# brucechin/OctopusZK

Measured on AMD Instinct MI355X. Metric: BN254 G1 VariableBaseMSM Mscalar-mul/s at 2^20, higher is better.
Workload: dtype u32; 1 GPU; VariableBaseMSM BN254 G1 2^20 random scalars/bases per GPU, bit-exact vs the serial CPU path (BASELINE.json configs[1]); n_per_gpu=1048576, window_bits=16, windows=8, glv=True, prepared_bases=False, msms_in_flight=3, schedule=pipeline3, parallelism=index-range shard x1, RCCL all-gather of 192-B partials + HIP point sum

## Files before the change

### octopuszk_amd/csrc/msm_var.cuh

```cuda
#pragma once
#include "curve.cuh"
#include "glv.cuh"

namespace ozk {

constexpr u32 BID_NONE = 0xffffffffu;

struct MsmPlan {
  int n_in;
  int glv;
  int n;
  int sd;
  int c;
  int cb;
  int W;
  int L1;
  int LK;
  int S;
};

OZK_HD u32 scalar_digit(const u32 (&s)[8], int w, int c) {
  const int bit = w * c;
  const int wi = bit >> 5, sh = bit & 31;
  u32 v = s[wi] >> sh;
// ... 693 lines not shown
    return IO::load_aff(w);
  }
  __device__ __forceinline__ void start_signed(const Aff<EA>& q, bool negate) {
    Aff<EA> qs = q;
    qs.y = select_el(negate, EA(reduce_to<17>(neg(q.y))), q.y);
    a = xyzz_from_affine<CV>(qs);
  }
  __device__ __forceinline__ void accumulate_signed(const Aff<EA>& q, bool negate) { a = xyzz_madd_lazy(a, q, negate); }
  __device__ __forceinline__ void store(u32* dst) const { IO::store_rec_xyzz(a, dst); }
  __device__ __forceinline__ void negate() { a.Y = typename CV::XY(reduce_to<32>(neg(reduce_to<32>(a.Y)))); }
  __device__ __forceinline__ void store_infinity(u32* dst) const {
    Xyzz<CV> z = a;
    z.ZZ = typename CV::XZZ(el_zero(z.ZZ));
    z.ZZZ = typename CV::XZZZ(el_zero(z.ZZ));
    IO::store_rec_xyzz(z, dst);
  }
};

template <class CV>
struct RunAccLds {
  using IO = CurveIO<CV>;
  using EA = typename CV::EA;
  static constexpr int RW = IO::RW;
  static constexpr int LDS_WORDS = 4 * RW;
  u32* col;
  template <class E>
  __device__ __forceinline__ E ld(int c) const {
    u32 w[RW];
#pragma unroll
    for (int k = 0; k < RW; k++) w[k] = col[(size_t)(c * RW + k) * 256];
    return ElemTraits<E>::load_raw(w);
  }
  template <class E>
  __device__ __forceinline__ void st(int c, const E& e) const {
    u32 w[RW];
    ElemTraits<E>::store_raw(e, w);
#pragma unroll
    for (int k = 0; k < RW; k++) col[(size_t)(c * RW + k) * 256] = w[k];
  }
  __device__ __forceinline__ void init(u32* lds) { col = lds + threadIdx.x; }
  __device__ __forceinline__ void put(const Xyzz<CV>& a) const {
    st(0, a.X);
    st(1, a.Y);
    st(2, a.ZZ);
    st(3, a.ZZZ);
  }
  static __device__ __forceinline__ Aff<EA> load_signed(const u32* pts, const u32* idx, long long p) {
    return RunAcc<CV, true>::load_signed(pts, idx, p);
  }
  using Raw = typename RunAcc<CV, true>::Raw;
  static __device__ __forceinline__ Raw load_raw(const u32* pts, u32 v) { return RunAcc<CV, true>::load_raw(pts, v); }
  static __device__ __forceinline__ __amdgpu_buffer_rsrc_t table_rsrc(const u32* pts) { return RunAcc<CV, true>::table_rsrc(pts); }
  static __device__ __forceinline__ Raw load_raw_buf(__amdgpu_buffer_rsrc_t rs, u32 v) { return RunAcc<CV, true>::load_raw_buf(rs, v); }
  static __device__ __forceinline__ Aff<EA> decode(const Raw& r, u32 v) { return RunAcc<CV, true>::decode(r, v); }
  __device__ __forceinline__ void start(const u32* pts, const u32* idx, long long p) {
    start_q(load_signed(pts, idx, p));
  }
  __device__ __forceinline__ void accumulate(const u32* pts, const u32* idx, long long p) {
    accumulate_q(load_signed(pts, idx, p));
  }
  __device__ __forceinline__ void start_q(const Aff<EA>& q) { put(xyzz_from_affine<CV>(q)); }
  __device__ __forceinline__ void accumulate_q(const Aff<EA>& q) {
    if (is_inf(q)) return;
    const auto ZZ = ld<typename CV::XZZ>(2);
    if (is_zero(ZZ)) {
      put(xyzz_from_affine<CV>(q));
      return;
    }
    if constexpr (CV::LAZY_FQ2) {
      const auto U2 = mul_lz(q.x, ZZ);
      const auto P = sub(U2, ld<typename CV::XX>(0));
      const auto ZZZ = ld<typename CV::XZZZ>(3);
      const auto R = sub(mul_lz(q.y, ZZZ), ld<typename CV::XY>(1));
      if (is_zero(P)) {
        if (is_zero(R)) {
          put(xyzz_dbl_affine<CV>(q));
        } else {
          st(2, typename CV::XZZ(el_zero(q.x)));
          st(3, typename CV::XZZZ(el_zero(q.x)));
        }
        return;
      }
      const auto Pr = reduce_to<32>(P);
      const auto PP = sqr_lz(Pr);
      const auto PPP = mul_lz(Pr, PP);
      st(2, typename CV::XZZ(mul_lz(ZZ, PP)));
      st(3, typename CV::XZZZ(mul_lz(ZZZ, PPP)));
      asm volatile("" ::: "memory");
      const auto Q = mul_lz(reduce_to<32>(ld<typename CV::XX>(0)), PP);
      const auto X3 = sub_sub2(sqr_lz(reduce_to<32>(R)), PPP, Q);
      st(0, typename CV::XX(X3));
      asm volatile("" ::: "memory");
      const auto Y3 = mulsub_lz(reduce_to<32>(R), reduce_to<32>(sub(Q, X3)), ld<typename CV::XY>(1), PPP);
      st(1, typename CV::XY(Y3));
      return;
    }
    const auto U2 = mul(q.x, ZZ);
    const auto P = sub(U2, ld<typename CV::XX>(0));
    const auto ZZZ = ld<typename CV::XZZZ>(3);
    const auto R = sub(mul(q.y, ZZZ), ld<typename CV::XY>(1));
    if (is_zero(P)) {
      if (is_zero(R)) {
        put(xyzz_dbl_affine<CV>(q));
      } else {
        st(2, typename CV::XZZ(el_zero(q.x)));
        st(3, typename CV::XZZZ(el_zero(q.x)));
      }
      return;
    }
    const auto PP = sqr(P);
    const auto PPP = mul(P, PP);
    st(2, typename CV::XZZ(mul(ZZ, PP)));
    st(3, typename CV::XZZZ(mul(ZZZ, PPP)));
    asm volatile("" ::: "memory");
    const auto Q = mul(ld<typename CV::XX>(0), PP);
    const auto X3 = sub(sqr(R), add(PPP, dbl(Q)));
    st(0, typename CV::XX(X3));
    asm volatile("" ::: "memory");
    const auto Y3 = mulsub(R, sub(Q, X3), ld<typename CV::XY>(1), PPP);
    st(1, typename CV::XY(Y3));
  }
  __device__ __forceinline__ Xyzz<CV> get() const {
    Xyzz<CV> a;
    a.X = ld<typename CV::XX>(0);
    a.Y = ld<typename CV::XY>(1);
    a.ZZ = ld<typename CV::XZZ>(2);
    a.ZZZ = ld<typename CV::XZZZ>(3);
    return a;
  }
  __device__ __forceinline__ void store(u32* dst) const { IO::store_rec_xyzz(get(), dst); }
  __device__ __forceinline__ void negate() const {
    st(1, typename CV::XY(reduce_to<32>(neg(reduce_to<32>(ld<typename CV::XY>(1))))));
  }
  __device__ __forceinline__ void store_infinity(u32* dst) const {
    Xyzz<CV> z = get();
    z.ZZ = typename CV::XZZ(el_zero(z.ZZ));
    z.ZZZ = typename CV::XZZZ(el_zero(z.ZZ));
    IO::store_rec_xyzz(z, dst);
  }
};
template <class CV>
struct RunAcc<CV, false> {
  using IO = CurveIO<CV>;
  Jac<CV> a;
  __device__ __forceinline__ void start(const u32* pts, const u32*, long long p) {
    a = IO::load_rec(pts + (size_t)p * IO::REC_WORDS);
  }
  __device__ __forceinline__ void accumulate(const u32* pts, const u32*, long long p) {
    a = jac_add(a, IO::load_rec(pts + (size_t)p * IO::REC_WORDS));
  }
  __device__ __forceinline__ void store(u32* dst) const { IO::store_rec_jac(a, dst); }
};

template <class CV, bool FIRST, bool LAZY = false>
__device__ __forceinline__ void
segreduce_lane(const int t, const u32* __restrict__ bid_in, const u32* __restrict__ idx_in,
               const u32* __restrict__ pts_in,
               const u32* __restrict__ d_count, int n_in_static, int L,
               u32* __restrict__ buckets, u32* __restrict__ bid_out, u32* __restrict__ pts_out) {
  using IO = CurveIO<CV>;
  if (!FIRST && *d_count == 0) return;
  const long long n_in = FIRST ? (long long)(*d_count) : (long long)n_in_static;
  const uint2* ent = reinterpret_cast<const uint2*>(idx_in);
  auto bid_at = [&](long long p) -> u32 {
    if constexpr (FIRST) return ent[p].y;
    else return bid_in[p];
  };
  const long long s = (long long)t * L;
  u32 head_bid = BID_NONE, tail_bid = BID_NONE;
  bool live = s < n_in;
  if (!FIRST && live) {
    const long long e0 = (s + L < n_in) ? (s + L) : n_in;
    bool any = false;
    for (long long p = s; p < e0; p++) any = any || (bid_in[p] != BID_NONE);
    live = any;
  }
  if (live) {
    const long long e = (s + L < n_in) ? (s + L) : n_in;
    const u32 first_bid = bid_at(s);
    const bool cb = (s > 0) && (bid_at(s - 1) == first_bid) && (first_bid != BID_NONE);
    const u32 last_bid = bid_at(e - 1);
    const bool cf = (e < n_in) && (bid_at(e) == last_bid) && (last_bid != BID_NONE);
    u32 cur = BID_NONE;
    bool cur_cb = false;
    using Acc = std::conditional_t<(FIRST && CV::LDS_ACC), RunAccLds<CV>, RunAcc<CV, FIRST>>;
    Acc acc;
    if constexpr (FIRST && CV::LDS_ACC) {
      extern __shared__ u32 ozk_acc_lds[];
      acc.init(ozk_acc_lds);
    }
    if constexpr (FIRST) {
      const u32 n_e = (u32)(e - s);
      const uint2* ent_c = ent + s;
      const uint2 e_first = ent_c[0];
      uint2 e_next = ent_c[n_e > 1 ? 1 : 0];
      u32 v_cur = e_first.x;
      const __amdgpu_buffer_rsrc_t table = Acc::table_rsrc(pts_in);
      typename Acc::Raw r = Acc::load_raw_buf(table, v_cur);
      u32 b_cur = first_bid;
      for (u32 k = 0; k < n_e; k++) {
        const u32 b = b_cur;
        const bool negate = (v_cur & SIDX_NEG) != 0;
        const auto q = [&] {
          if constexpr (LAZY) return Acc::decode_unsigned(r);
          else return Acc::decode(r, v_cur);
        }();
        const u32 k2 = (k + 2 < n_e) ? k + 2 : n_e - 1;
        const uint2 en = e_next;
        r = Acc::load_raw_buf(table, en.x);
        b_cur = en.y;
        v_cur = en.x;
        e_next = ent_c[k2];
        if (b != cur) {
          if (cur != BID_NONE) {
            if (cur_cb) {
              head_bid = cur;
              acc.store(pts_out + (size_t)(2 * (size_t)t) * IO::REC_WORDS);
            } else {
              acc.store(buckets + (size_t)cur * IO::REC_WORDS);
            }
          }
          cur = b;
          cur_cb = (k == 0) && cb;
          if constexpr (LAZY) acc.start_signed(q, negate);
          else acc.start_q(q);
        } else {
          if constexpr (LAZY) acc.accumulate_signed(q, negate);
          else acc.accumulate_q(q);
        }
      }
    } else {
    for (long long p = s; p < e; p++) {
      const u32 b = bid_in[p];
      if (b != cur) {
        if (cur != BID_NONE) {
          if (cur_cb) {
            head_bid = cur;
            acc.store(pts_out + (size_t)(2 * (size_t)t) * IO::REC_WORDS);
          } else {
            acc.store(buckets + (size_t)cur * IO::REC_WORDS);
          }
        }
        cur = b;
        cur_cb = (p == s) && cb;
        if (b != BID_NONE) acc.start(pts_in, idx_in, p);
      } else if (b != BID_NONE) {
        acc.accumulate(pts_in, idx_in, p);
      }
    }
    }
    if (cur != BID_NONE) {
      if (cur_cb) {
        head_bid = cur;
        acc.store(pts_out + (size_t)(2 * (size_t)t) * IO::REC_WORDS);
        if (cf) {
          tail_bid = cur;
          if constexpr (FIRST) {
            acc.store_infinity(pts_out + (size_t)(2 * (size_t)t + 1) * IO::REC_WORDS);
          } else {
            IO::store_rec_jac(jac_infinity<CV>(), pts_out + (size_t)(2 * (size_t)t + 1) * IO::REC_WORDS);
          }
        }
      } else if (cf) {
        tail_bid = cur;
        acc.store(pts_out + (size_t)(2 * (size_t)t + 1) * IO::REC_WORDS);
      } else {
        acc.store(buckets + (size_t)cur * IO::REC_WORDS);
      }
    }
  }
  bid_out[2 * (size_t)t] = head_bid;
  bid_out[2 * (size_t)t + 1] = tail_bid;
}

template <class CV, bool FIRST, bool LAZY = false>
__global__ void __launch_bounds__(256, (FIRST && CV::LDS_ACC) ? 2 : 1)
k_segreduce(const u32* __restrict__ bid_in, const u32* __restrict__ idx_in, const u32* __restrict__ pts_in,
            const u32* __restrict__ d_count, int n_in_static, int L,
            u32* __restrict__ buckets, u32* __restrict__ bid_out, u32* __restrict__ pts_out,
            int n_lanes, unsigned long long* __restrict__ clk) {
  const int t = blockIdx.x * blockDim.x + threadIdx.x;
  unsigned long long w0 = 0, c0 = 0;
  if constexpr (FIRST) {
    if (clk != nullptr && threadIdx.x == 0) {
      w0 = (unsigned long long)wall_clock64();
      c0 = (unsigned long long)clock64();
      atomicMax(&clk[0], ~w0);
    }
  }
  if (t < n_lanes)
    segreduce_lane<CV, FIRST, LAZY>(t, bid_in, idx_in, pts_in, d_count, n_in_static, L, buckets, bid_out, pts_out);
  if constexpr (FIRST) {
    if (clk != nullptr && (threadIdx.x & 63) == 0) {
      const unsigned long long w1 = (unsigned long long)wall_clock64();
      atomicMax(&clk[1], w1);
      if (threadIdx.x == 0) {
        atomicAdd(&clk[2], (unsigned long long)clock64() - c0);
        atomicAdd(&clk[3], w1 - w0);
      }
    }
  }
}

static __global__ void k_read_clock(unsigned long long* out) { out[0] = (unsigned long long)wall_clock64(); }

template <class CV>
__global__ void __launch_bounds__(256)
k_segreduce_small(const u32* __restrict__ d_count, int n_in, int L, u32* __restrict__ buckets,
                  u32* __restrict__ bid_a, u32* __restrict__ pts_a, u32* __restrict__ bid_b, u32* __restrict__ pts_b) {
  if (*d_count == 0) return;
  u32 *bi = bid_a, *pi = pts_a, *bo = bid_b, *po = pts_b;
  while (true) {
    const int lanes = (n_in + L - 1) / L;
    for (int t = threadIdx.x; t < lanes; t += blockDim.x)
      segreduce_lane<CV, false>(t, bi, nullptr, pi, d_count, n_in, L, buckets, bo, po);
    if (lanes == 1) break;
    block_sync();
    n_in = 2 * lanes;
    u32* tb = bi; bi = bo; bo = tb;
    u32* tp = pi; pi = po; po = tp;
  }
}

constexpr int RUN_MAX = 16;
template <class CV>
__global__ void __launch_bounds__(256)
k_runmerge(const u32* __restrict__ bid_in, const u32* __restrict__ pts, int n_slots,
           u32* __restrict__ buckets, u32* __restrict__ bid_out, u32* __restrict__ remaining) {
  using IO = CurveIO<CV>;
  const int t = blockIdx.x * blockDim.x + threadIdx.x;
  u32 alive = 0;
#pragma unroll 1
  for (int k = 0; k < 2; k++) {
    const int x = 2 * t + 1 + k;
    if (x >= n_slots) break;
    const u32 bx = bid_in[x];
    u32 out = BID_NONE;
    if (bx != BID_NONE) {
      int s = x, e = x;
      while (s > 0 && x - s < RUN_MAX && bid_in[s - 1] == bx) s--;
      while (e + 1 < n_slots && e - x < RUN_MAX && bid_in[e + 1] == bx) e++;
      const bool is_short = (x - s < RUN_MAX) && (e - x < RUN_MAX) && (e - s + 1 <= RUN_MAX);
      if (!is_short) {
        out = bx;
      } else if (s == x) {
        Xyzz<CV> acc = IO::load_xyzz(pts + (size_t)s * IO::REC_WORDS);
        for (int q = s + 1; q <= e; q += 2) acc = xyzz_add(acc, IO::load_xyzz(pts + (size_t)q * IO::REC_WORDS));
        IO::store_rec_xyzz(acc, buckets + (size_t)bx * IO::REC_WORDS);
      }
    }
    bid_out[x] = out;
    alive += (out != BID_NONE);
  }
  if (t == 0 && n_slots > 0) {
    bid_out[0] = bid_in[0];
    alive += (bid_in[0] != BID_NONE);
  }
  for (int o = 32; o > 0; o >>= 1) alive += __shfl_xor(alive, o);
  if ((threadIdx.x & 63) == 0 && alive) atomicAdd(remaining, alive);
}

template <class CV, bool FIRSTLEVEL>
__global__ void __launch_bounds__(256)
k_wsum(const u32* __restrict__ A_in, const u32* __restrict__ R_in, const u32* __restrict__ hist,
       int m_in, int S, int g, u32* __restrict__ A_out, u32* __restrict__ R_out, int m_out, int W, int prio) {
  using IO = CurveIO<CV>;
  if (prio) __builtin_amdgcn_s_setprio(3);
  const int t = blockIdx.x * blockDim.x + threadIdx.x;
  if (t >= m_out * W) return;
  const int w = t / m_out, j = t - w * m_out;
  const size_t base = (size_t)w * m_in;
  const int lo = j * S;
  int hi = lo + S;
  if (hi > m_in) hi = m_in;
  Jac<CV> run = jac_infinity<CV>(), ws = jac_infinity<CV>(), asum = jac_infinity<CV>();
  for (int e = hi - 1; e >= lo; e--) {
    if constexpr (FIRSTLEVEL) {
      if (hist[base + e] != 0) run = jac_add(run, IO::load_rec(R_in + (base + e) * IO::REC_WORDS));
    } else {
      run = jac_add(run, IO::load_jac(R_in + (base + e) * IO::JAC_WORDS));
    }
    if (e > lo) ws = jac_add(ws, run);
    if constexpr (!FIRSTLEVEL) asum = jac_add(asum, IO::load_jac(A_in + (base + e) * IO::JAC_WORDS));
  }
  for (int k = 0; k < g; k++) ws = jac_dbl(ws);
  if constexpr (!FIRSTLEVEL) ws = jac_add(ws, asum);
  IO::store_jac(ws, A_out + ((size_t)w * m_out + j) * IO::JAC_WORDS);
  IO::store_jac(run, R_out + ((size_t)w * m_out + j) * IO::JAC_WORDS);
}

template <class CV>
__device__ __forceinline__ Jac<CV> shfl_down_jac(const Jac<CV>& p, int o) {
  Jac<CV> r;
  r.X = shfl_down_el(p.X, o);
  r.Y = shfl_down_el(p.Y, o);
  r.Z = shfl_down_el(p.Z, o);
  return r;
}

template <class CV>
__device__ __forceinline__ void wave_combine(Jac<CV>& A, Jac<CV>& T, int l, int valid, int g) {
  for (int o = 1; o < valid; o <<= 1) {
    const Jac<CV> t = shfl_down_jac(T, o);
    const Jac<CV> s = jac_add(T, t);
    if (l + o < 64) T = s;
  }
  Jac<CV> U = T;
  for (int k = 0; k < g; k++) U = jac_dbl(U);
  const Jac<CV> AV = jac_add(A, U);
  Jac<CV> V = (l >= 1) ? AV : A;
  int top = 1;
  while (top < valid) top <<= 1;
  for (int o = top >> 1; o > 0; o >>= 1) {
    const Jac<CV> v = shfl_down_jac(V, o);
    const Jac<CV> s = jac_add(V, v);
    if (l < o) V = s;
  }
  A = V;
}

template <class CV>
__global__ void __launch_bounds__(64)
k_wsum_wave(const u32* __restrict__ A_in, const u32* __restrict__ R_in, int m_in, int g,
            u32* __restrict__ A_out, u32* __restrict__ R_out, int m_out, int W) {
  using IO = CurveIO<CV>;
  __builtin_amdgcn_s_setprio(3);
  const int wave = blockIdx.x;
  if (wave >= m_out * W) return;
  const int w = wave / m_out, j = wave - w * m_out;
  const int l = threadIdx.x & 63;
  const int e = j * 64 + l;
  int valid = m_in - j * 64;
  if (valid > 64) valid = 64;
  Jac<CV> A = jac_infinity<CV>(), T = jac_infinity<CV>();
  if (e < m_in) {
    A = IO::load_jac(A_in + ((size_t)w * m_in + e) * IO::JAC_WORDS);
    T = IO::load_jac(R_in + ((size_t)w * m_in + e) * IO::JAC_WORDS);
  }
  wave_combine<CV>(A, T, l, valid, g);
  if (l == 0) {
    IO::store_jac(A, A_out + ((size_t)w * m_out + j) * IO::JAC_WORDS);
    IO::store_jac(T, R_out + ((size_t)w * m_out + j) * IO::JAC_WORDS);
  }
}

template <class CV>
__global__ void __launch_bounds__(64)
k_wsum_fused(const u32* __restrict__ buckets, const u32* __restrict__ hist, int m_in, int S, int sg,
             u32* __restrict__ A_out, u32* __restrict__ R_out, int m_out, int W, int prio) {
  using IO = CurveIO<CV>;
  if (prio) __builtin_amdgcn_s_setprio(3);
  const int wave = blockIdx.x;
// ... 210 lines not shown
```

### octopuszk_amd/csrc/msm_var_driver.cuh

```cuda
#pragma once
#include <hip/hip_ext.h>
#include <pthread.h>
#include <stdlib.h>

#include <atomic>
#include <vector>

#ifndef OZK_WITH_G2
#define OZK_WITH_G2 1
#endif
#include "msm_var.cuh"
#include "host_ctx.h"
#include "fq2.cuh"

namespace ozk {

enum { PROF_OFF = 0, PROF_EVENTS = 1, PROF_CLOCK = 2 };
struct ProfState {
  pthread_mutex_t mu = PTHREAD_MUTEX_INITIALIZER;
  std::atomic<int> mode{PROF_OFF};
  int src = PROF_EVENTS;
  int every = 1, seen = 0;
  int count = 0;
  std::vector<hipEvent_t> e0, e1;
// ... 206 lines not shown
    rb->sorted = (a.off + 255) & ~(size_t)255;
    rb->sort_ws = (b.off + 255) & ~(size_t)255;
    rb->accum_ws = (c.off + 255) & ~(size_t)255;
  }
  L.bytes = a.off + b.off + c.off;
  return L;
}
template <class CV>
RegionBytes region_bytes(int n) {
  RegionBytes rb;
  make_layout3<CV>(plan_for<CV>(n), nullptr, nullptr, nullptr, &rb);
  return rb;
}

template <class CV>
size_t tail_layout(const MsmPlan& p, MsmLayout& L, void* tail, size_t tail_bytes) {
  using IO = CurveIO<CV>;
  Bump b(tail, tail_bytes);
  L.NB = (size_t)p.W << p.cb;
  L.m1 = (((size_t)1 << p.cb) + p.S - 1) / p.S;
  L.buckets = b.take<u32>(L.NB * IO::REC_WORDS);
  L.hist_t = b.take<u32>(L.NB);
  for (int k = 0; k < 2; k++) {
    L.wA[k] = b.take<u32>((size_t)p.W * L.m1 * IO::JAC_WORDS);
    L.wR[k] = b.take<u32>((size_t)p.W * L.m1 * IO::JAC_WORDS);
  }
  b.take<u32>(64);
  return b.off;
}

enum { TAIL_LATENCY = 0, TAIL_THROUGHPUT = 1 };
struct TailShape {
  bool fused;
  int serial_above;
};
static TailShape tail_shape(int mode) {
  const int forced = env_int("OZK_MSM_TAIL_MODE", -1);
  if (forced == 0 || forced == 1) mode = forced;
  TailShape t;
  t.fused = env_int("OZK_MSM_WSUM_FUSED", mode == TAIL_THROUGHPUT ? 0 : 1) != 0;
  t.serial_above = env_int("OZK_MSM_TAIL_SERIAL_ABOVE", mode == TAIL_THROUGHPUT ? 64 : (1 << 30));
  return t;
}
static void first_level_shape(const MsmPlan& p, bool fused, int* m_out, int* g_out) {
  const int m_in = 1 << p.cb;
  const int nseg = (m_in + p.S - 1) / p.S;
  const int sg = ilog2((uint32_t)p.S);
  if (fused) {
    *m_out = (nseg + 63) / 64;
    *g_out = sg + 6;
  } else {
    *m_out = nseg;
    *g_out = sg;
  }
}
template <class CV>
void launch_wsum0(const MsmPlan& p, const MsmLayout& L, hipStream_t st, int prio, bool fused) {
  const int TB = 256;
  const int m_in = 1 << p.cb;
  int m_out, g;
  first_level_shape(p, fused, &m_out, &g);
  const int tot = m_out * p.W;
  if (fused)
    hipLaunchKernelGGL((k_wsum_fused<CV>), dim3(tot), dim3(64), 0, st, L.buckets, L.hist_t, m_in, p.S,
                       ilog2((uint32_t)p.S), L.wA[0], L.wR[0], m_out, p.W, prio);
  else
    hipLaunchKernelGGL((k_wsum<CV, true>), dim3((tot + TB - 1) / TB), dim3(TB), 0, st, (const u32*)nullptr,
                       L.buckets, L.hist_t, m_in, p.S, 0, L.wA[0], L.wR[0], m_out, p.W, prio);
}

template <class CV>
int var_msm_sort(const void* d_bases, const void* d_scalars, int n, void* sorted, size_t sorted_bytes,
                        void* sort_ws, size_t sort_ws_bytes, hipStream_t st, hipEvent_t order_ev = nullptr,
                        const void* prepared = nullptr) {
  hip_clear_stale();
  const MsmPlan p = plan_for<CV>(n);
  if (prepared && p.glv && !p.sd) return fail(OZK_E_INVALID, "prepared bases need the signed-digit plan");
  RegionBytes rb;
  const MsmLayout L = make_layout3<CV>(p, sorted, sort_ws, nullptr, &rb, prepared);
  if (rb.sorted > sorted_bytes || rb.sort_ws > sort_ws_bytes)
    return fail(OZK_E_INVALID, "sort buffers too small: need %zu + %zu bytes, got %zu + %zu", rb.sorted, rb.sort_ws,
                sorted_bytes, sort_ws_bytes);
  const int TB = 256;
  const u32* bases = (const u32*)d_bases;
  const u32* scalars = (const u32*)d_scalars;
  const int n_in = p.n_in;
  n = p.n;
  OZK_HIP(hipMemsetAsync(L.total, 0, 4 * sizeof(u32), st));
  if (p.glv) {
    hipLaunchKernelGGL(k_digits_glv, dim3((n_in + TB - 1) / TB), dim3(TB), 0, st, scalars, n_in, p.c, p.W, p.sd,
                       L.digits, L.neg_flags);
    if (!prepared)
      hipLaunchKernelGGL((k_convert_bases<CV>), dim3((n_in + TB - 1) / TB), dim3(TB), 0, st, bases, L.aff, n_in, 1,
                         p.sd ? (const uint8_t*)nullptr : (const uint8_t*)L.neg_flags);
  } else {
    if (!prepared)
      hipLaunchKernelGGL((k_convert_bases<CV>), dim3((n_in + TB - 1) / TB), dim3(TB), 0, st, bases, L.aff, n_in, 0,
                         (const uint8_t*)nullptr);
    hipLaunchKernelGGL(k_digits, dim3((n_in + TB - 1) / TB), dim3(TB), 0, st, scalars, n_in, p.c, p.W, L.digits);
  }
  if (n <= SORTS_MAX_N && p.cb <= SORTS_MAX_CB && env_int("OZK_MSM_SMALL_SORT", 1)) {
    hipLaunchKernelGGL(k_sort_small, dim3(p.W), dim3(SORTS_BLOCK), 0, st, L.digits, n, p.cb, p.sd, L.total, L.hist, L.sent);
    if (order_ev && env_int("OZK_MSM_ORDER", 1)) OZK_HIP(hipStreamWaitEvent(st, order_ev, 0));
    OZK_HIP(hipGetLastError());
    return OZK_OK;
  }
  const size_t lds1 = (size_t)L.NH * sizeof(u32);
  hipLaunchKernelGGL(k_sort1_count, dim3(L.nblk, p.W), dim3(SORT_BLOCK), lds1, st, L.digits, n, L.lo_bits, p.sd,
                     L.NH, L.nblk, L.C1);
  const int items = SCAN_BLOCK * SCAN_ITEMS;
  const int nb = (int)((L.nC1 + items - 1) / items);
  hipLaunchKernelGGL(k_scan_blocksum, dim3(nb), dim3(SCAN_BLOCK), 0, st, L.C1, (int)L.nC1, L.blocksum);
  hipLaunchKernelGGL(k_scan_top, dim3(1), dim3(1024), 0, st, L.blocksum, nb, L.total);
  hipLaunchKernelGGL(k_scan_final, dim3(nb), dim3(SCAN_BLOCK), 0, st, L.C1, (int)L.nC1, L.blocksum, L.P1);
  const size_t lds_sc = ((size_t)2 * L.NH + 2 * SORT_CHUNK) * sizeof(u32);
  hipLaunchKernelGGL(k_sort1_scatter, dim3(L.nblk, p.W), dim3(SORT_BLOCK), lds_sc, st, L.digits, n, L.lo_bits,
                     p.sd, L.NH, L.nblk, L.P1, L.total, L.nC1, L.coarse);
  const int nbins = p.W * L.NH;
  const u32 sign_bit = p.sd ? 0x80u : 0u;
  const u32 big_thresh = (u32)(n / 64) > SORT_BIG ? (u32)(n / 64) : SORT_BIG;
  if (L.cap / ((size_t)big_thresh + 1) > (size_t)SORTBIG_MAXBINS)
    return fail(OZK_E_INVALID, "window plan c=%d (W=%d) at n=%d can produce more than %d oversized sort bins",
                p.c, p.W, p.n_in, SORTBIG_MAXBINS);
  hipLaunchKernelGGL(k_sort2, dim3(nbins), dim3(SORT2_BLOCK), 0, st, L.coarse, L.P1, L.total, p.cb, L.lo_bits, L.NH,
                     sign_bit, L.nblk, nbins, big_thresh, L.hist, L.sent);
  if (order_ev && env_int("OZK_MSM_ORDER", 1)) OZK_HIP(hipStreamWaitEvent(st, order_ev, 0));
  hipLaunchKernelGGL(k_sortbig_list, dim3(1), dim3(256), 0, st, L.P1, L.total, L.nblk, nbins, big_thresh, L.bigbins);
  hipLaunchKernelGGL(k_sortbig_count, dim3(1024), dim3(SORT_BLOCK), 0, st, L.coarse, L.bigbins,
                     (1u << L.lo_bits) - 1u, L.bigT);
  hipLaunchKernelGGL(k_sortbig_scan, dim3(SORTBIG_MAXBINS), dim3(256), 0, st, L.bigbins, L.bigT, p.cb, L.lo_bits, L.NH,
                     L.hist);
  hipLaunchKernelGGL(k_sortbig_scatter, dim3(1024), dim3(SORT_BLOCK), 0, st, L.coarse, L.bigbins, L.bigT, p.cb,
                     L.lo_bits, sign_bit, L.NH, L.sent);
  OZK_HIP(hipGetLastError());
  return OZK_OK;
}

enum { ACCUM_ALL = 0, ACCUM_LEVEL1 = 1, ACCUM_REST = 2 };
template <class CV>
int var_msm_accum(int n, void* sorted, size_t sorted_bytes, void* accum_ws, size_t accum_ws_bytes, void* tail,
                         size_t tail_bytes, hipStream_t st, const void* prepared = nullptr, int part = ACCUM_ALL) {
  hip_clear_stale();
  using CT = CV;
  const MsmPlan p = plan_for<CV>(n);
  RegionBytes rb;
  MsmLayout L = make_layout3<CV>(p, sorted, nullptr, accum_ws, &rb, prepared);
  if (rb.sorted > sorted_bytes || rb.accum_ws > accum_ws_bytes)
    return fail(OZK_E_INVALID, "accumulate buffers too small: need %zu + %zu bytes, got %zu + %zu", rb.sorted,
                rb.accum_ws, sorted_bytes, accum_ws_bytes);
  const size_t tneed = tail_layout<CV>(p, L, tail, tail_bytes);
  if (tneed > tail_bytes) return fail(OZK_E_INVALID, "tail buffer too small: need %zu bytes, got %zu", tneed, tail_bytes);
  const int TB = 256;
  size_t lanes = (L.cap + p.L1 - 1) / p.L1;
  if (part != ACCUM_REST) {
  hipEvent_t prof_e0 = nullptr, prof_e1 = nullptr;
  unsigned long long* clk = nullptr;
  g_prof.claim(&prof_e0, &prof_e1, &clk);
  const bool prof = prof_e0 != nullptr;
  size_t acc_lds = CV::LDS_ACC ? (size_t)RunAccLds<CV>::LDS_WORDS * TB * sizeof(u32) : 0;
  if (!CV::LDS_ACC) acc_lds = (size_t)env_int("OZK_L1_LDS", 41216);
  auto launch_l1 = [&](auto kern) {
    if (acc_lds > 65536)
      OZK_HIP(hipFuncSetAttribute((const void*)kern, hipFuncAttributeMaxDynamicSharedMemorySize, (int)acc_lds));
    hipExtLaunchKernelGGL(kern, dim3((unsigned)((lanes + TB - 1) / TB)), dim3(TB), (uint32_t)acc_lds, st,
                          prof ? prof_e0 : (hipEvent_t) nullptr, prof ? prof_e1 : (hipEvent_t) nullptr, 0u,
                          (const u32*)nullptr, (const u32*)L.sent, (const u32*)L.aff, (const u32*)L.total, 0, p.L1,
                          L.buckets, L.slot_bid[0], L.slot_pts[0], (int)lanes, clk);
    return OZK_OK;
  };
  int rc_l1;
  if constexpr (CV::LAZY_MADD) {
    if (env_int("OZK_L1_LAZY", 1)) rc_l1 = launch_l1(k_segreduce<CV, true, true>);
    else rc_l1 = launch_l1(k_segreduce<CV, true, false>);
  } else {
    rc_l1 = launch_l1(k_segreduce<CV, true, false>);
  }
  if (rc_l1) return rc_l1;
  }
  if (part == ACCUM_LEVEL1) {
    OZK_HIP(hipGetLastError());
    return OZK_OK;
  }
  size_t n_in = 2 * lanes;
  hipLaunchKernelGGL((k_runmerge<CT>), dim3((unsigned)((lanes + TB - 1) / TB)), dim3(TB), 0, st, L.slot_bid[0],
                     L.slot_pts[0], (int)n_in, L.buckets, L.slot_bid2, L.total + 1);
  int cur = 0;
  bool first_generic = true;
  const int small_lanes = env_int("OZK_MSM_SMALL_LEVEL_LANES", 1024);
  while (true) {
    lanes = (n_in + p.LK - 1) / p.LK;
    if (!first_generic && (int)lanes <= small_lanes) {
      hipLaunchKernelGGL((k_segreduce_small<CT>), dim3(1), dim3(TB), 0, st, L.total + 1, (int)n_in, p.LK, L.buckets,
                         L.slot_bid[cur], L.slot_pts[cur], L.slot_bid[cur ^ 1], L.slot_pts[cur ^ 1]);
      break;
    }
    hipLaunchKernelGGL((k_segreduce<CT, false>), dim3((unsigned)((lanes + TB - 1) / TB)), dim3(TB), 0, st,
                       first_generic ? L.slot_bid2 : L.slot_bid[cur], (const u32*)nullptr, L.slot_pts[cur],
                       L.total + 1, (int)n_in, p.LK, L.buckets, L.slot_bid[cur ^ 1], L.slot_pts[cur ^ 1], (int)lanes,
                       (unsigned long long*)nullptr);
    first_generic = false;
    if (lanes == 1) break;
    n_in = 2 * lanes;
    cur ^= 1;
  }
  OZK_HIP(hipMemcpyAsync(L.hist_t, L.hist, L.NB * sizeof(u32), hipMemcpyDeviceToDevice, st));
  OZK_HIP(hipGetLastError());
  return OZK_OK;
}

template <class CV>
int var_msm_head(const void* d_bases, const void* d_scalars, int n, void* ws, size_t ws_bytes, void* tail,
                        size_t tail_bytes, hipStream_t st, hipEvent_t order_ev = nullptr,
                        const void* prepared = nullptr) {
  const RegionBytes rb = region_bytes<CV>(n);
  if (rb.sorted + rb.sort_ws + rb.accum_ws > ws_bytes)
    return fail(OZK_E_INVALID, "workspace too small: need %zu bytes, got %zu", rb.sorted + rb.sort_ws + rb.accum_ws,
                ws_bytes);
  uint8_t* w = (uint8_t*)ws;
  int rc = var_msm_sort<CV>(d_bases, d_scalars, n, w, rb.sorted, w + rb.sorted, rb.sort_ws, st, order_ev, prepared);
  if (rc) return rc;
  return var_msm_accum<CV>(n, w, rb.sorted, w + rb.sorted + rb.sort_ws, rb.accum_ws, tail, tail_bytes, st, prepared);
}

template <class CV>
int var_msm_tail(int n, void* tail, size_t tail_bytes, void* d_out, hipStream_t st,
                        hipEvent_t order_ev = nullptr, int mode = TAIL_LATENCY) {
  hip_clear_stale();
  using CT = CV;
  MsmPlan p = plan_for<CV>(n);
  MsmLayout L;
  L.m1 = (((size_t)1 << p.cb) + p.S - 1) / p.S;
  const size_t tneed = tail_layout<CV>(p, L, tail, tail_bytes);
  if (tneed > tail_bytes) return fail(OZK_E_INVALID, "tail buffer too small: need %zu bytes, got %zu", tneed, tail_bytes);
  const TailShape shape = tail_shape(mode);
  if (shape.fused && mode == TAIL_LATENCY) {
    int s_dflt = p.S;
    if (std::is_same<CV, G1Cfg>::value && p.cb >= 13) s_dflt = 8;
    const int s_lat = env_int("OZK_MSM_S_LAT", s_dflt);
    if (s_lat >= 2 && s_lat <= 64) p.S = 1 << ilog2((uint32_t)s_lat);
  }
  launch_wsum0<CV>(p, L, st, env_int("OZK_MSM_WSUM0_PRIO", 0), shape.fused);
  int m_in, g, k = 0;
  first_level_shape(p, shape.fused, &m_in, &g);
  const int TB = 256;
  const int sg = ilog2((uint32_t)p.S);
  const int serial_above = shape.serial_above < 1 ? 1 : shape.serial_above;
  while (m_in > serial_above) {
    const int m_out = (m_in + p.S - 1) / p.S;
    const int tot = m_out * p.W;
    hipLaunchKernelGGL((k_wsum<CT, false>), dim3((tot + TB - 1) / TB), dim3(TB), 0, st, L.wA[k], L.wR[k],
                       (const u32*)nullptr, m_in, p.S, g, L.wA[k ^ 1], L.wR[k ^ 1], m_out, p.W, 1);
    m_in = m_out;
    g += sg;
    k ^= 1;
  }
  int fin_max = env_int("OZK_MSM_FIN_MAX", 4);
  if (fin_max < 1) fin_max = 1;
  if (fin_max > 16) fin_max = 16;
  const bool order_early = env_int("OZK_MSM_ORDER_EARLY", 1) != 0;
  if (order_ev && order_early) OZK_HIP(hipEventRecord(order_ev, st));
  while (m_in > fin_max) {
    const int m_out = (m_in + 63) / 64;
    const int tot = m_out * p.W;
    hipLaunchKernelGGL((k_wsum_wave<CT>), dim3(tot), dim3(64), 0, st, L.wA[k], L.wR[k], m_in, g, L.wA[k ^ 1],
                       L.wR[k ^ 1], m_out, p.W);
    m_in = m_out;
    g += 6;
    k ^= 1;
  }
  if (order_ev && !order_early) OZK_HIP(hipEventRecord(order_ev, st));
  hipLaunchKernelGGL((k_finalize<CT>), dim3(1), dim3(64), 0, st, L.wA[k], L.wR[k], m_in, g, p.W, p.c, p.sd,
                     (u32*)d_out);
  OZK_HIP(hipGetLastError());
  return OZK_OK;
}

template <class CV>
size_t var_msm_tail_bytes(int n) {
  const MsmPlan p = plan_for<CV>(n);
  MsmLayout L;
  L.m1 = (((size_t)1 << p.cb) + p.S - 1) / p.S;
  return tail_layout<CV>(p, L, nullptr, 0);
}

template <class CV>
int var_msm_dev(const void* d_bases, const void* d_scalars, int n, void* d_out, void* ws,
                       size_t ws_bytes, hipStream_t st, const void* prepared = nullptr) {
  LonePlan lone;
  const RegionBytes rb0 = region_bytes<CV>(n);
  const size_t main_bytes = rb0.sorted + rb0.sort_ws + rb0.accum_ws;
  const size_t tb = var_msm_tail_bytes<CV>(n);
  if (main_bytes + tb > ws_bytes)
    return fail(OZK_E_INVALID, "workspace too small: need %zu bytes, got %zu", main_bytes + tb, ws_bytes);
  uint8_t* tail = (uint8_t*)ws + main_bytes;
  int rc = var_msm_head<CV>(d_bases, d_scalars, n, ws, main_bytes, tail, tb, st, nullptr, prepared);
  if (rc) return rc;
  return var_msm_tail<CV>(n, tail, tb, d_out, st);
}

template <class CV>
size_t var_msm_head_ws_bytes(int n) {
  const RegionBytes rb = region_bytes<CV>(n);
  return rb.sorted + rb.sort_ws + rb.accum_ws;
}
template <class CV>
size_t var_msm_ws_bytes(int n) {
  return var_msm_head_ws_bytes<CV>(n) + var_msm_tail_bytes<CV>(n);
}

inline int host_slices(int n) {
  int kmax = env_int("OZK_HOST_SLICES", 8);
  if (kmax > MAX_SLICES) kmax = MAX_SLICES;
  int min_log = env_int("OZK_HOST_SLICE_MIN_LOG", 18);
  if (min_log < 4) min_log = 4;
  if (min_log > 30) min_log = 30;
  int k = n >> min_log;
  if (k > kmax) k = kmax;
  return k < 1 ? 1 : k;
}

inline int host_slice_per(int n, int K) {
  if (K < 2) return n;
  if (env_int("OZK_HOST_SLICE_TAPER", 1) == 0) return (n + K - 1) / K;
  const long long rest = (long long)n - (long long)n / (2 * K);
  return (int)((rest + K - 2) / (K - 1));
}
static bool plans_agree(int n1, int n2) {
  const MsmPlan a = make_plan(n1), b = make_plan(n2);
  return a.c == b.c && a.cb == b.cb && a.W == b.W && a.sd == b.sd && a.glv == b.glv && a.S == b.S;
}

template <class CV>
size_t host_sliced_ws_bytes(int K, int per) {
  return pad256(var_msm_head_ws_bytes<CV>(per)) + (size_t)K * pad256(var_msm_tail_bytes<CV>(per));
}
template <class CV>
int host_sliced_msm(HostCtx* c, const uint8_t* bases, const uint8_t* scalars, int n, int K, int per, uint8_t* d_bases,
                    uint8_t* d_sc, uint8_t* d_ws, uint8_t* d_out, hipEvent_t* ev, hipStream_t st, hipStream_t up) {
  hip_clear_stale();
  using IO = CurveIO<CV>;
  const size_t base_rec = (size_t)IO::WIRE_JAC_WORDS * 4;
// ... 210 lines not shown
```

Before: 724.7 Mscalar-mul/s.

## Merge level-1 segment-reduce boundary partials inside each block via LDS

Adds a level-1 segmented-reduce kernel that keeps each lane's head partial in LDS and merges cross-lane bucket runs within the 256-thread block, so each block writes only two boundary partials instead of two per lane. It also folds the histogram copy into this kernel, and the later reduction levels start from per-block rather than per-lane partials. The aim is to cut global traffic and the number and size of subsequent merge levels. The cost is extra LDS use, block syncs and serial run-chasing by leader lanes, which can lower occupancy.

```diff
diff --git a/octopuszk_amd/csrc/msm_var.cuh b/octopuszk_amd/csrc/msm_var.cuh
--- a/octopuszk_amd/csrc/msm_var.cuh
+++ b/octopuszk_amd/csrc/msm_var.cuh
@@ -869,12 +869,42 @@
   __device__ __forceinline__ void store(u32* dst) const { IO::store_rec_jac(a, dst); }
 };
 
-template <class CV, bool FIRST, bool LAZY = false>
+template <class CV>
+__device__ __forceinline__ void lds_put_xyzz(u32* col, const Xyzz<CV>& a) {
+  using IO = CurveIO<CV>;
+  u32 w[4 * IO::RW];
+  ElemTraits<typename CV::XX>::store_raw(a.X, w);
+  ElemTraits<typename CV::XY>::store_raw(a.Y, w + IO::RW);
+  ElemTraits<typename CV::XZZ>::store_raw(a.ZZ, w + 2 * IO::RW);
+  ElemTraits<typename CV::XZZZ>::store_raw(a.ZZZ, w + 3 * IO::RW);
+#pragma unroll
+  for (int k = 0; k < 4 * IO::RW; k++) col[k * 256] = w[k];
+}
+template <class CV>
+__device__ __forceinline__ Xyzz<CV> lds_get_xyzz(const u32* col) {
+  using IO = CurveIO<CV>;
+  u32 w[4 * IO::RW];
+#pragma unroll
+  for (int k = 0; k < 4 * IO::RW; k++) w[k] = col[k * 256];
+  return IO::load_xyzz(w);
+}
+
+template <class CV>
+struct L1Edge {
+  u32 head_bid = BID_NONE;
+  u32 tail_bid = BID_NONE;
+  bool full = false;
+  Xyzz<CV> tail;
+};
+
+template <class CV, bool FIRST, bool LAZY = false, bool BM = false>
 __device__ __forceinline__ void
 segreduce_lane(const int t, const u32* __restrict__ bid_in, const u32* __restrict__ idx_in,
                const u32* __restrict__ pts_in,
                const u32* __restrict__ d_count, int n_in_static, int L,
-               u32* __restrict__ buckets, u32* __restrict__ bid_out, u32* __restrict__ pts_out) {
+               u32* __restrict__ buckets, u32* __restrict__ bid_out, u32* __restrict__ pts_out,
+               L1Edge<CV>* edge = nullptr, u32* head_col = nullptr) {
+  static_assert(!BM || (FIRST && !CV::LDS_ACC), "the block merge is a level-1 form of the register accumulator");
   using IO = CurveIO<CV>;
   if (!FIRST && *d_count == 0) return;
   const long long n_in = FIRST ? (long long)(*d_count) : (long long)n_in_static;
@@ -932,7 +962,8 @@
           if (cur != BID_NONE) {
             if (cur_cb) {
               head_bid = cur;
-              acc.store(pts_out + (size_t)(2 * (size_t)t) * IO::REC_WORDS);
+              if constexpr (BM) lds_put_xyzz<CV>(head_col, acc.a);
+              else acc.store(pts_out + (size_t)(2 * (size_t)t) * IO::REC_WORDS);
             } else {
               acc.store(buckets + (size_t)cur * IO::REC_WORDS);
             }
@@ -966,6 +997,25 @@
       }
     }
     }
+    if constexpr (BM) {
+      if (cur != BID_NONE) {
+        if (cur_cb) {
+          head_bid = cur;
+          lds_put_xyzz<CV>(head_col, acc.a);
+          if (cf) {
+            tail_bid = cur;
+            edge->full = true;
+            edge->tail = acc.a;
+            edge->tail.ZZ = typename CV::XZZ(el_zero(acc.a.ZZ));
+          }
+        } else if (cf) {
+          tail_bid = cur;
+          edge->tail = acc.a;
+        } else {
+          acc.store(buckets + (size_t)cur * IO::REC_WORDS);
+        }
+      }
+    } else
     if (cur != BID_NONE) {
       if (cur_cb) {
         head_bid = cur;
@@ -986,8 +1036,13 @@
       }
     }
   }
-  bid_out[2 * (size_t)t] = head_bid;
-  bid_out[2 * (size_t)t + 1] = tail_bid;
+  if constexpr (BM) {
+    edge->head_bid = head_bid;
+    edge->tail_bid = tail_bid;
+  } else {
+    bid_out[2 * (size_t)t] = head_bid;
+    bid_out[2 * (size_t)t + 1] = tail_bid;
+  }
 }
 
 template <class CV, bool FIRST, bool LAZY = false>
@@ -1015,6 +1070,94 @@
         atomicAdd(&clk[2], (unsigned long long)clock64() - c0);
         atomicAdd(&clk[3], w1 - w0);
       }
+    }
+  }
+}
+
+constexpr int L1M_GROUP = 16;
+template <class CV>
+constexpr size_t l1m_lds_bytes() { return ((size_t)4 * CurveIO<CV>::RW * 256 + 8) * sizeof(u32); }
+template <class CV, bool LAZY>
+__global__ void __launch_bounds__(256)
+k_segreduce_l1m(const u32* __restrict__ idx_in, const u32* __restrict__ pts_in, const u32* __restrict__ d_count, int L,
+                u32* __restrict__ buckets, u32* __restrict__ bid_out, u32* __restrict__ pts_out, int n_lanes,
+                const u32* __restrict__ hist, u32* __restrict__ hist_t, int n_hist, unsigned long long* __restrict__ clk) {
+  using IO = CurveIO<CV>;
+  static_assert(L1M_GROUP == 16, "run_end reads one 16-bit field of the mask");
+  extern __shared__ u32 ozk_l1m_lds[];
+  u32* const heads = ozk_l1m_lds;
+  u32* const fullm = ozk_l1m_lds + 4 * IO::RW * 256;
+  const int u = threadIdx.x;
+  const int t = blockIdx.x * blockDim.x + u;
+  unsigned long long w0 = 0, c0 = 0;
+  if (clk != nullptr && u == 0) {
+    w0 = (unsigned long long)wall_clock64();
+    c0 = (unsigned long long)clock64();
+    atomicMax(&clk[0], ~w0);
+  }
+  for (long long i = t; i < n_hist; i += (long long)gridDim.x * blockDim.x) hist_t[i] = hist[i];
+  L1Edge<CV> ed;
+  if (t < n_lanes)
+    segreduce_lane<CV, true, LAZY, true>(t, nullptr, idx_in, pts_in, d_count, 0, L, buckets, nullptr, nullptr, &ed,
+                                         heads + u);
+  const unsigned long long fb = __ballot(ed.full);
+  if ((u & 63) == 0) {
+    fullm[u >> 5] = (u32)fb;
+    fullm[(u >> 5) + 1] = (u32)(fb >> 32);
+  }
+  block_sync();
+  auto is_full = [&](int v) -> bool { return (fullm[v >> 5] >> (v & 31)) & 1u; };
+  auto jumps = [&](int g) -> bool { return (g % L1M_GROUP) == 0 && is_full(g) && is_full(g + 1); };
+  auto run_end = [&](int g) -> int {
+    const u32 nf = ~(fullm[g >> 5] >> (g & 31)) & 0xffffu;
+    return nf ? g + __builtin_ctz(nf) : g + L1M_GROUP - 1;
+  };
+  const size_t hs = 2 * (size_t)blockIdx.x, ts = hs + 1;
+  const bool has_tail = ed.tail_bid != BID_NONE && !ed.full;
+  const bool cut_start = u == 0 && ed.full;
+  if (u == 0 && ed.head_bid != BID_NONE && !ed.full)
+    IO::store_rec_xyzz(lds_get_xyzz<CV>(heads), pts_out + hs * IO::REC_WORDS);
+  Xyzz<CV> a = ed.tail;
+  const bool lead = jumps(u);
+  if (lead) {
+    const int v = run_end(u);
+    for (int k = u; k <= v; k++) a = xyzz_add(a, lds_get_xyzz<CV>(heads + k));
+    lds_put_xyzz<CV>(heads + u, a);
+  }
+  block_sync();
+  int cur = cut_start ? (lead ? run_end(0) : -1) : u;
+  bool go = has_tail || (cut_start && (!lead || is_full(cur)));
+  bool open = false;
+  while (go) {
+    if (cur == 255) {
+      open = true;
+      break;
+    }
+    const int nx = cur + 1;
+    a = xyzz_add(a, lds_get_xyzz<CV>(heads + nx));
+    cur = jumps(nx) ? run_end(nx) : nx;
+    go = is_full(cur);
+  }
+  if (has_tail || cut_start) {
+    if (open) {
+      IO::store_rec_xyzz(a, pts_out + (cut_start ? hs : ts) * IO::REC_WORDS);
+      if (cut_start) {
+        a.ZZ = typename CV::XZZ(el_zero(a.ZZ));
+        a.ZZZ = typename CV::XZZZ(el_zero(a.ZZ));
+        IO::store_rec_xyzz(a, pts_out + ts * IO::REC_WORDS);
+      }
+    } else {
+      IO::store_rec_xyzz(a, cut_start ? pts_out + hs * IO::REC_WORDS : buckets + (size_t)ed.tail_bid * IO::REC_WORDS);
+    }
+  }
+  if (u == 0) bid_out[hs] = ed.head_bid;
+  if (u == 255) bid_out[ts] = ed.tail_bid;
+  if (clk != nullptr && (u & 63) == 0) {
+    const unsigned long long w1 = (unsigned long long)wall_clock64();
+    atomicMax(&clk[1], w1);
+    if (u == 0) {
+      atomicAdd(&clk[2], (unsigned long long)clock64() - c0);
+      atomicAdd(&clk[3], w1 - w0);
     }
   }
 }
diff --git a/octopuszk_amd/csrc/msm_var_driver.cuh b/octopuszk_amd/csrc/msm_var_driver.cuh
--- a/octopuszk_amd/csrc/msm_var_driver.cuh
+++ b/octopuszk_amd/csrc/msm_var_driver.cuh
@@ -382,6 +382,8 @@
   if (tneed > tail_bytes) return fail(OZK_E_INVALID, "tail buffer too small: need %zu bytes, got %zu", tneed, tail_bytes);
   const int TB = 256;
   size_t lanes = (L.cap + p.L1 - 1) / p.L1;
+  const bool merge = !CV::LDS_ACC && env_int("OZK_L1_MERGE", 1) != 0;
+  const size_t l1_blocks = (lanes + TB - 1) / TB;
   if (part != ACCUM_REST) {
   hipEvent_t prof_e0 = nullptr, prof_e1 = nullptr;
   unsigned long long* clk = nullptr;
@@ -398,16 +400,62 @@
                           L.buckets, L.slot_bid[0], L.slot_pts[0], (int)lanes, clk);
     return OZK_OK;
   };
-  int rc_l1;
-  if constexpr (CV::LAZY_MADD) {
-    if (env_int("OZK_L1_LAZY", 1)) rc_l1 = launch_l1(k_segreduce<CV, true, true>);
-    else rc_l1 = launch_l1(k_segreduce<CV, true, false>);
-  } else {
-    rc_l1 = launch_l1(k_segreduce<CV, true, false>);
+  int rc_l1 = OZK_OK;
+  if constexpr (!CV::LDS_ACC) {
+    if (merge) {
+      acc_lds = std::max(acc_lds, l1m_lds_bytes<CV>());
+      auto launch_l1m = [&](auto kern) {
+        if (acc_lds > 65536)
+          OZK_HIP(hipFuncSetAttribute((const void*)kern, hipFuncAttributeMaxDynamicSharedMemorySize, (int)acc_lds));
+        hipExtLaunchKernelGGL(kern, dim3((unsigned)l1_blocks), dim3(TB), (uint32_t)acc_lds, st,
+                              prof ? prof_e0 : (hipEvent_t) nullptr, prof ? prof_e1 : (hipEvent_t) nullptr, 0u,
+                              (const u32*)L.sent, (const u32*)L.aff, (const u32*)L.total, p.L1, L.buckets,
+                              L.slot_bid[0], L.slot_pts[0], (int)lanes, (const u32*)L.hist, L.hist_t, (int)L.NB, clk);
+        return OZK_OK;
+      };
+      if (env_int("OZK_L1_LAZY", 1)) rc_l1 = launch_l1m(k_segreduce_l1m<CV, true>);
+      else rc_l1 = launch_l1m(k_segreduce_l1m<CV, false>);
+    }
+  }
+  if (!merge) {
+    if constexpr (CV::LAZY_MADD) {
+      if (env_int("OZK_L1_LAZY", 1)) rc_l1 = launch_l1(k_segreduce<CV, true, true>);
+      else rc_l1 = launch_l1(k_segreduce<CV, true, false>);
+    } else {
+      rc_l1 = launch_l1(k_segreduce<CV, true, false>);
+    }
   }
   if (rc_l1) return rc_l1;
   }
   if (part == ACCUM_LEVEL1) {
+    OZK_HIP(hipGetLastError());
+    return OZK_OK;
+  }
+  const int small_lanes = env_int("OZK_MSM_SMALL_LEVEL_LANES", 1024);
+  if (merge) {
+    size_t n_in = 2 * l1_blocks;
+    u32 *bid_a = L.slot_bid[0], *pts_a = L.slot_pts[0], *bid_b = L.slot_bid[1], *pts_b = L.slot_pts[1];
+    const u32* count = L.total;
+    if (env_int("OZK_L1M_RUNMERGE", 1)) {
+      hipLaunchKernelGGL((k_runmerge<CT>), dim3((unsigned)((l1_blocks + TB - 1) / TB)), dim3(TB), 0, st, L.slot_bid[0],
+                         L.slot_pts[0], (int)n_in, L.buckets, L.slot_bid2, L.total + 1);
+      bid_a = L.slot_bid2;
+      count = L.total + 1;
+    }
+    while (true) {
+      lanes = (n_in + p.LK - 1) / p.LK;
+      if ((int)lanes <= small_lanes) {
+        hipLaunchKernelGGL((k_segreduce_small<CT>), dim3(1), dim3(TB), 0, st, count, (int)n_in, p.LK, L.buckets,
+                           bid_a, pts_a, bid_b, pts_b);
+        break;
+      }
+      hipLaunchKernelGGL((k_segreduce<CT, false>), dim3((unsigned)((lanes + TB - 1) / TB)), dim3(TB), 0, st, bid_a,
+                         (const u32*)nullptr, pts_a, count, (int)n_in, p.LK, L.buckets, bid_b, pts_b, (int)lanes,
+                         (unsigned long long*)nullptr);
+      n_in = 2 * lanes;
+      std::swap(bid_a, bid_b);
+      std::swap(pts_a, pts_b);
+    }
     OZK_HIP(hipGetLastError());
     return OZK_OK;
   }
@@ -416,7 +464,6 @@
                      L.slot_pts[0], (int)n_in, L.buckets, L.slot_bid2, L.total + 1);
   int cur = 0;
   bool first_generic = true;
-  const int small_lanes = env_int("OZK_MSM_SMALL_LEVEL_LANES", 1024);
   while (true) {
     lanes = (n_in + p.LK - 1) / p.LK;
     if (!first_generic && (int)lanes <= small_lanes) {
```

Measured after the change: 751.2 Mscalar-mul/s (median of 6 runs). 1.04x the previous value.
